# anihcsam/OpenGaussian

Measured on AMD Instinct MI355X. Metric: fwd+bwd Mpix/s at 1080p, 1M Gaussians (RGB+6-D ins_feat); k-means it/s, higher is better.
Workload: dtype f32; 1 GPU; S1M-1080p RGB(SH3)+depth+alpha (all grads) + 6-ch ins_feat (grad to ins_feat) fwd+bwd, ONE fused 9-channel pass; gaussians=1000000, width=1920, height=1080, views_cycled=8, parallelism=single

## Files before the change

include/ogs_raster.h:

```cpp
#ifndef OGS_RASTER_H
#define OGS_RASTER_H

#include <stddef.h>
#include <stdint.h>

#ifdef __cplusplus
extern "C" {
#endif

#define OGS_OK 0
#define OGS_ERR_INVALID_ARG (-1)
#define OGS_ERR_HIP (-2)
#define OGS_ERR_UNSUPPORTED (-3)
#define OGS_ERR_SCRATCH_TOO_SMALL (-4)
#define OGS_ERR_DEVICE (-5)

#define OGS_TILE 16
#define OGS_MAX_CHANNELS 12

typedef struct OgsRasterFwdArgs {
    int32_t P;
    int32_t W, H;
    int32_t C;
    int32_t sh_degree;
// ... 69 lines not shown
    float* dL_drotations;
    int32_t num_groups;
    float* dL_dsh_rgb;
    int32_t bwd_tmp_is_clear;
} OgsRasterBwdArgs;

int ogs_version(void);
const char* ogs_last_error(void);

int ogs_check_async_status(void);

size_t ogs_raster_geom_bytes(int32_t P, int32_t C);
size_t ogs_raster_geom_tmp_bytes(int32_t P);
size_t ogs_raster_image_bytes(int32_t W, int32_t H);
size_t ogs_raster_image_bytes_grouped(int32_t W, int32_t H, int32_t num_groups);
size_t ogs_raster_binning_tmp_bytes(int64_t num_rendered, int32_t W, int32_t H);
size_t ogs_raster_backward_tmp_bytes(int32_t P);
size_t ogs_raster_sorted_bytes(int64_t num_rendered, int32_t C);
size_t ogs_raster_quad_list_bytes(int64_t num_rendered);

int ogs_raster_forward_geometry(const OgsRasterFwdArgs* args, void* stream, int64_t* num_rendered_host);

int ogs_raster_forward_render(const OgsRasterFwdArgs* args, int64_t num_rendered, void* stream);

int ogs_raster_read_num_rendered_async(const OgsRasterFwdArgs* args, void* stream, uint32_t* host_pinned);
int ogs_raster_forward_render_deferred(const OgsRasterFwdArgs* args, int64_t capacity, void* stream);

int ogs_raster_read_num_emitted(const OgsRasterFwdArgs* args, void* stream, uint32_t* host);

size_t ogs_raster_tiny_max_points(void);
int ogs_raster_forward_tiny(const OgsRasterFwdArgs* args, void* stream);

size_t ogs_raster_tile_sort_capacity(int32_t level);

int ogs_raster_tile_count_debug(int64_t D, int64_t tiles, int32_t force_blocks, int32_t reverse);
size_t ogs_raster_tile_count_trip(void);

int ogs_raster_tile_place_debug(int64_t D, int64_t tiles, int32_t group, int32_t slices, int32_t stage_words, int32_t* chosen);

int ogs_raster_forward_reblend(const OgsRasterFwdArgs* args, void* stream);

int ogs_raster_compact_kept(int32_t W, int32_t H, int32_t C, const void* image_buffer, const void* sorted_rec,
                            const void* quad_list, void* new_image_buffer, void* new_sorted_rec, void* new_quad_list,
                            void* stream);

typedef struct OgsGroupStatsArgs {
    const int32_t* labels;
    int32_t num_labels;
    float alpha_threshold;
    float* max_alpha;
    int64_t* count;
    float* feat_sum;
    void* stats_tmp;
} OgsGroupStatsArgs;

size_t ogs_raster_stats_image_bytes(int32_t W, int32_t H, int32_t num_groups);
size_t ogs_raster_stats_tmp_bytes(int32_t num_groups, int32_t num_labels, int32_t C);
int ogs_raster_forward_group_stats(const OgsRasterFwdArgs* args, const OgsGroupStatsArgs* stats, int64_t num_rendered,
                                   void* stream);

int ogs_raster_backward(const OgsRasterBwdArgs* args, void* stream);

int ogs_mark_visible(int32_t P, const float* means3D, const float* viewmatrix, const float* projmatrix,
                     uint8_t* present, void* stream);

int ogs_sh_grad_from_views(int32_t P, int32_t V, int32_t sh_degree, int32_t sh_coeffs, const float* means3D,
// ... 23 lines not shown
```

opengaussian_amd/_lib.py:

```python
from __future__ import annotations

import ctypes as C
import os

_HERE = os.path.dirname(os.path.abspath(__file__))
LIB_PATH = os.environ.get("OGS_LIB_PATH") or os.path.join(_HERE, "lib", "libogs_hip.so")

_f32p = C.POINTER(C.c_float)
_vp = C.c_void_p


class OgsRasterFwdArgs(C.Structure):
    _fields_ = [
        ("P", C.c_int32), ("W", C.c_int32), ("H", C.c_int32), ("C", C.c_int32),
        ("sh_degree", C.c_int32), ("sh_coeffs", C.c_int32),
        ("tanfovx", C.c_float), ("tanfovy", C.c_float), ("scale_modifier", C.c_float),
        ("prefiltered", C.c_int32), ("debug", C.c_int32),
        ("bg", _vp), ("means3D", _vp), ("colors_precomp", _vp), ("shs", _vp), ("opacities", _vp),
        ("scales", _vp), ("rotations", _vp), ("cov3D_precomp", _vp),
        ("viewmatrix", _vp), ("projmatrix", _vp), ("campos", _vp),
        ("out_color", _vp), ("out_depth", _vp), ("out_alpha", _vp), ("radii", _vp),
        ("geom_buffer", _vp), ("geom_tmp", _vp), ("image_buffer", _vp), ("point_list", _vp),
        ("binning_tmp", _vp), ("sorted_rec", _vp), ("quad_list", _vp), ("group_ids", _vp), ("num_groups", C.c_int32),
        ("full_binning", C.c_int32),
# ... 57 lines not shown
                ("channels_last", C.c_int32), ("out_map", _vp), ("out_alpha", _vp)]


class OgsRawModel(C.Structure):
    _fields_ = [("features_dc", _vp), ("features_rest", _vp), ("scaling", _vp), ("rotation", _vp), ("opacity", _vp)]


class OgsRawModelGrads(C.Structure):
    _fields_ = [("features_dc", _vp), ("features_rest", _vp), ("scaling", _vp), ("rotation", _vp), ("opacity", _vp)]


SIGNATURES = {
    "ogs_version": (C.c_int, []),
    "ogs_last_error": (C.c_char_p, []),
    "ogs_raster_geom_bytes": (C.c_size_t, [C.c_int32, C.c_int32]),
    "ogs_raster_geom_tmp_bytes": (C.c_size_t, [C.c_int32]),
    "ogs_raster_image_bytes": (C.c_size_t, [C.c_int32, C.c_int32]),
    "ogs_raster_image_bytes_grouped": (C.c_size_t, [C.c_int32, C.c_int32, C.c_int32]),
    "ogs_raster_binning_tmp_bytes": (C.c_size_t, [C.c_int64, C.c_int32, C.c_int32]),
    "ogs_raster_backward_tmp_bytes": (C.c_size_t, [C.c_int32]),
    "ogs_raster_sorted_bytes": (C.c_size_t, [C.c_int64, C.c_int32]),
    "ogs_raster_quad_list_bytes": (C.c_size_t, [C.c_int64]),
    "ogs_raster_forward_geometry": (C.c_int, [C.POINTER(OgsRasterFwdArgs), _vp, C.POINTER(C.c_int64)]),
    "ogs_raster_forward_render": (C.c_int, [C.POINTER(OgsRasterFwdArgs), C.c_int64, _vp]),
    "ogs_raster_read_num_rendered_async": (C.c_int, [C.POINTER(OgsRasterFwdArgs), _vp, _vp]),
    "ogs_raster_forward_render_deferred": (C.c_int, [C.POINTER(OgsRasterFwdArgs), C.c_int64, _vp]),
    "ogs_raster_read_num_emitted": (C.c_int, [C.POINTER(OgsRasterFwdArgs), _vp, C.POINTER(C.c_uint32)]),
    "ogs_raster_stats_image_bytes": (C.c_size_t, [C.c_int32, C.c_int32, C.c_int32]),
    "ogs_raster_stats_tmp_bytes": (C.c_size_t, [C.c_int32, C.c_int32, C.c_int32]),
    "ogs_raster_forward_group_stats": (C.c_int, [C.POINTER(OgsRasterFwdArgs), C.POINTER(OgsGroupStatsArgs), C.c_int64, _vp]),
    "ogs_raster_backward": (C.c_int, [C.POINTER(OgsRasterBwdArgs), _vp]),
    "ogs_raster_tiny_max_points": (C.c_size_t, []),
    "ogs_raster_tile_sort_capacity": (C.c_size_t, [C.c_int32]),
    "ogs_raster_tile_count_debug": (C.c_int, [C.c_int64, C.c_int64, C.c_int32, C.c_int32]),
    "ogs_raster_tile_count_trip": (C.c_size_t, []),
    "ogs_raster_tile_place_debug": (C.c_int, [C.c_int64, C.c_int64, C.c_int32, C.c_int32, C.c_int32, C.POINTER(C.c_int32)]),
    "ogs_raster_forward_tiny": (C.c_int, [C.POINTER(OgsRasterFwdArgs), _vp]),
    "ogs_raster_forward_reblend": (C.c_int, [C.POINTER(OgsRasterFwdArgs), _vp]),
    "ogs_raster_compact_kept": (C.c_int, [C.c_int32, C.c_int32, C.c_int32, _vp, _vp, _vp, _vp, _vp, _vp, _vp]),
    "ogs_mark_visible": (C.c_int, [C.c_int32, _vp, _vp, _vp, _vp, _vp]),
    "ogs_sh_grad_from_views": (C.c_int, [C.c_int32, C.c_int32, C.c_int32, C.c_int32, _vp, _vp, _vp, _vp, _vp]),
    "ogs_raster_export_binning": (C.c_int, [C.POINTER(OgsRasterFwdArgs), C.c_int64, _vp, _vp, _vp, _vp]),
    "ogs_selftest_wave_fold16": (C.c_int, [_vp, _vp, _vp]),
    "ogs_selftest_mfma_rank1": (C.c_int, [_vp, _vp, _vp, C.c_int32, _vp, _vp, _vp]),
    "ogs_selftest_tile_order": (C.c_int, [_vp, C.c_int64, _vp, _vp]),
    "ogs_selftest_radix_tmp_bytes": (C.c_size_t, [C.c_int64]),
    "ogs_selftest_radix_sort": (C.c_int, [_vp, _vp, _vp, _vp, C.c_int64, C.c_int32, C.c_int32, C.c_int32, _vp, _vp, _vp, _vp]),
    "ogs_raster_forward_geometry_raw": (C.c_int, [C.POINTER(OgsRasterFwdArgs), C.POINTER(OgsRawModel), _vp,
                                                  C.POINTER(C.c_int64)]),
    "ogs_raster_forward_tiny_raw": (C.c_int, [C.POINTER(OgsRasterFwdArgs), C.POINTER(OgsRawModel), _vp]),
    "ogs_raster_backward_raw": (C.c_int, [C.POINTER(OgsRasterBwdArgs), C.POINTER(OgsRawModel), C.POINTER(OgsRawModelGrads), _vp]),
    "ogs_model_activate": (C.c_int, [C.c_int32, C.c_int32, C.POINTER(OgsRawModel), _vp, _vp, _vp, _vp, _vp]),
    "ogs_check_async_status": (C.c_int, []),
    "ogs_prof_enable": (C.c_int, [C.c_int]),
    "ogs_prof_filter": (C.c_int, [C.c_char_p]),
    "ogs_prof_collect": (C.c_int, [C.c_char_p, C.c_size_t]),
    "ogs_kmeans_tmp_bytes": (C.c_size_t, [C.c_int64, C.c_int32, C.c_int32]),
    "ogs_kmeans_lloyd": (C.c_int, [_vp, C.c_int64, C.c_int32, _vp, C.c_int32, C.c_int32, C.c_int32, C.c_int32,
                                   _vp, C.c_int64, _vp, _vp]),
    "ogs_kmeans_assign": (C.c_int, [_vp, C.c_int64, C.c_int32, _vp, C.c_int32, _vp, C.c_int64, _vp]),
    "ogs_mask_feature_sums": (C.c_int, [_vp, _vp, _vp, C.c_int32, C.c_int32, C.c_int64, C.c_int32, _vp, _vp]),
    "ogs_mask_feature_sqdev": (C.c_int, [_vp, _vp, _vp, _vp, C.c_int32, C.c_int32, C.c_int64, _vp, _vp]),
    "ogs_mask_feature_sums_backward": (C.c_int, [_vp, _vp, _vp, _vp, _vp, C.c_int32, C.c_int32, C.c_int64, _vp, _vp, _vp]),
    "ogs_mask_cohesion": (C.c_int, [_vp, _vp, _vp, C.c_int32, C.c_int32, C.c_int64, _vp, _vp]),
    "ogs_mask_cohesion_backward": (C.c_int, [_vp, _vp, _vp, _vp, C.c_int32, C.c_int32, C.c_int64, _vp, _vp, _vp]),
    "ogs_label_feature_sums": (C.c_int, [_vp, _vp, _vp, C.c_int32, C.c_int32, C.c_int64, C.c_int32, _vp, _vp]),
# ... 151 lines not shown
```

opengaussian_amd/csrc/binning.hip:

```cpp
#include <stdlib.h>
#include <string.h>

#include <atomic>

#include "ogs_common.h"

namespace ogs {

namespace {

constexpr size_t kSweepHeaderWords = 4 * 256 + 4 + 60;
constexpr int kScanItems = 8;
constexpr int kScanTile = kBlock * kScanItems;

__device__ __forceinline__ uint32_t wave_inclusive_scan(uint32_t v) {
#pragma unroll
    for (int d = 1; d < kWave; d <<= 1) {
        uint32_t t = __shfl_up(v, d, kWave);
        if (lane_id() >= d) v += t;
    }
    return v;
}

__device__ __forceinline__ uint32_t block_exclusive_scan(uint32_t v, uint32_t& total, uint32_t* wave_sums ) {
    const int wave = threadIdx.x >> 6;
    const uint32_t inc = wave_inclusive_scan(v);
    if (lane_id() == kWave - 1) wave_sums[wave] = inc;
    __syncthreads();
    uint32_t base = 0, tot = 0;
#pragma unroll
    for (int w = 0; w < kBlock / kWave; ++w) {
        const uint32_t s = wave_sums[w];
// ... 613 lines not shown
        run_mine += c;
    }
    if (p == 0 && blockIdx.y == gridDim.y - 1 && threadIdx.x == 0) *kept = total;
    if (begin >= end || nt == 0 || (may_stage && need == 0)) return;
    __syncthreads();
    for (int j = threadIdx.x; j < nt; j += kCountBlock) (staged ? delta : cur)[j] += row[j];
    __syncthreads();
    const uint32_t ulo = (uint32_t)t_lo, unt = (uint32_t)nt;
    uint16_t* stile = reinterpret_cast<uint16_t*>(stage + stage_words);
    if (!staged) {
        tile_place_walk<false>(keys, vals, begin, end, reverse, ulo, unt, cur, stage, stile, stage_words, out, out_cap);
        return;
    }
    tile_place_walk<true>(keys, vals, begin, end, reverse, ulo, unt, cur, stage, stile, stage_words, out, out_cap);
    __syncthreads();
    for (uint32_t i = threadIdx.x; i < need; i += kCountBlock) {
        const uint32_t pos = delta[min((int)stile[i], nt - 1)] + i;
        if (pos < out_cap) out[pos] = stage[i];
    }
}

constexpr int kTileSortWaves = kBlock / kWave;
struct TileSortLds {
    uint32_t hist[kTileSortWaves][256];
    uint32_t dig_start[256];
    uint32_t base[256];
    uint32_t scan_sums[4];
    uint32_t red[2];
    uint2 range[kTileSortWaves];
    uint32_t kv[2 * kTileSortCap];
};
typedef __attribute__((address_space(3))) volatile uint32_t LdsWord;
typedef __attribute__((address_space(3))) unsigned long long LdsMask;
__device__ __forceinline__ LdsWord* lds_words(uint32_t* p) { return (LdsWord*)p; }
__device__ __forceinline__ LdsMask* wave_masks(TileSortLds& sm, int wave) { return (LdsMask*)(sm.kv + wave * 2 * kWaveSortCap); }

__device__ __forceinline__ void wave_rank_clear(LdsWord* hist, LdsMask* masks) {
    const int lane = threadIdx.x & (kWave - 1);
#pragma unroll
    for (int j = 0; j < 4; ++j) {
        hist[lane + j * kWave] = 0u;
        __hip_atomic_store(&masks[lane + j * kWave], 0ull, __ATOMIC_SEQ_CST, __HIP_MEMORY_SCOPE_WAVEFRONT);
    }
    __builtin_amdgcn_wave_barrier();
}

__device__ __forceinline__ void wave_rank(LdsWord* hist, LdsMask* masks, const uint32_t (&key)[kTileSortItems],
                                          uint32_t (&rank)[kTileSortItems], int ipl, int first, int m, int shift,
                                          uint32_t mask) {
    const int lane = threadIdx.x & (kWave - 1);
    const unsigned long long me = 1ull << lane;
#pragma unroll
    for (int i = 0; i < kTileSortItems; ++i) {
        if (i >= ipl) continue;
        const bool valid = first + i * kWave + lane < m;
        const uint32_t d = (key[i] >> shift) & mask;
        if (valid) __hip_atomic_fetch_or(&masks[d], me, __ATOMIC_SEQ_CST, __HIP_MEMORY_SCOPE_WAVEFRONT);
        __builtin_amdgcn_wave_barrier();
        const unsigned long long peers =
            valid ? __hip_atomic_load(&masks[d], __ATOMIC_SEQ_CST, __HIP_MEMORY_SCOPE_WAVEFRONT) : 0ull;
        const uint32_t r = __builtin_amdgcn_mbcnt_hi((uint32_t)(peers >> 32), __builtin_amdgcn_mbcnt_lo((uint32_t)peers, 0u));
        uint32_t pre = 0;
        if (valid) pre = hist[d];
        __builtin_amdgcn_wave_barrier();
        if (valid && r == 0) {
            hist[d] = pre + (uint32_t)__popcll(peers);
// ... 79 lines not shown
#pragma unroll
        for (int j = 0; j < 4; ++j) { c[j] = hist[4 * lane + j]; sum += c[j]; }
        uint32_t run = wave_inclusive_scan(sum) - sum;
#pragma unroll
        for (int j = 0; j < 4; ++j) { hist[4 * lane + j] = run; run += c[j]; }
        __builtin_amdgcn_wave_barrier();
#pragma unroll
        for (int i = 0; i < kTileSortItems; ++i) {
            if (i >= ipl) continue;
            rank[i] += hist[(sel[i] >> shift) & mask];
        }
#pragma unroll
        for (int i = 0; i < kTileSortItems; ++i) {
            if (i >= ipl) continue;
            if (i * kWave + lane < n) {
                wk[rank[i]] = key[i];
                wv[rank[i]] = val[i];
            }
        }
        __builtin_amdgcn_wave_barrier();
        if (p + 1 < npass || reload_last) {
#pragma unroll
            for (int i = 0; i < kTileSortItems; ++i) {
                if (i >= ipl) continue;
                const int e = min(i * kWave + lane, n - 1);
                key[i] = wk[e];
                val[i] = wv[e];
            }
            __builtin_amdgcn_wave_barrier();
        }
    }
}

__device__ __forceinline__ void wave_sort_list(TileSortLds& sm, uint32_t* __restrict__ seg, int n,
                                               const uint32_t* __restrict__ depth_keys) {
    const int lane = threadIdx.x & (kWave - 1), wave = threadIdx.x >> 6;
    LdsWord* wk = lds_words(sm.kv + wave * 2 * kWaveSortCap);
    LdsWord* wv = wk + kWaveSortCap;
    LdsWord* hist = lds_words(sm.hist[wave]);
    LdsMask* masks = wave_masks(sm, wave);
    uint32_t key[kTileSortItems], val[kTileSortItems], rank[kTileSortItems];
    const int ipl = (n + kWave - 1) / kWave;
    load_items(seg, depth_keys, key, val, ipl, lane, n);
    uint32_t k_and, k_or;
    wave_and_or(key, ipl, 0xFFFFFFFFu, k_and, k_or);
    const uint32_t kdiff = (uint32_t)__builtin_amdgcn_readfirstlane((int)(k_and ^ k_or));
    if (kdiff != 0u) {
        wave_lsd_passes(hist, masks, wk, wv, key, key, val, rank, ipl, n, kdiff, false);
    } else {
#pragma unroll
        for (int i = 0; i < kTileSortItems; ++i) {
            if (i >= ipl) continue;
            if (i * kWave + lane < n) { wk[i * kWave + lane] = key[i]; wv[i * kWave + lane] = val[i]; }
        }
        __builtin_amdgcn_wave_barrier();
    }
    bool bad = false;
#pragma unroll
    for (int i = 0; i < kTileSortItems; ++i) {
        if (i >= ipl) continue;
        const int e = min(i * kWave + lane, n - 2);
        if (wk[e] == wk[e + 1]) bad |= (wv[e] & kGidMask) > (wv[e + 1] & kGidMask);
    }
    if (__ballot(bad) != 0ull) {
#pragma unroll
        for (int i = 0; i < kTileSortItems; ++i) {
            if (i >= ipl) continue;
            const int e = min(i * kWave + lane, n - 1);
            key[i] = wk[e];
            val[i] = wv[e];
        }
        __builtin_amdgcn_wave_barrier();
        wave_and_or(val, ipl, kGidMask, k_and, k_or);
        const uint32_t gdiff = (uint32_t)__builtin_amdgcn_readfirstlane((int)(k_and ^ k_or));
        if (gdiff != 0u) wave_lsd_passes(hist, masks, wk, wv, val, key, val, rank, ipl, n, gdiff, kdiff != 0u);
        if (kdiff != 0u) wave_lsd_passes(hist, masks, wk, wv, key, key, val, rank, ipl, n, kdiff, false);
    } else if (kdiff == 0u) {
        return;
    }
// ... 161 lines not shown
            return;
        }
        for (int j = tid; j < n; j += kBlock) seg[j] = sv[j];
        return;
    }

    uint32_t k_and = 0xFFFFFFFFu, k_or = 0u;
    for (int j = tid; j < n; j += kBlock) {
        const uint32_t k = depth_keys[seg[j] & kGidMask];
        k_and &= k;
        k_or |= k;
    }
    const uint32_t kdiff = block_and_or(sm, k_and, k_or, any);
    if (kdiff != 0u) long_lsd_passes<false>(sm, seg, alt, n, depth_keys, kdiff);
    bool bad = false;
    k_and = 0xFFFFFFFFu; k_or = 0u;
    for (int j = tid; j < n; j += kBlock) {
        const uint32_t v0 = seg[j], v1 = seg[min(j + 1, n - 1)];
        bad |= tie_out_of_order(depth_keys[v0 & kGidMask], v0, depth_keys[v1 & kGidMask], v1);
        k_and &= v0 & kGidMask;
        k_or |= v0 & kGidMask;
    }
    const uint32_t gdiff = block_and_or(sm, k_and, k_or | (bad ? 0x80000000u : 0u), any) & kGidMask;
    if ((any & 0x80000000u) == 0u || gdiff == 0u) return;
    long_lsd_passes<true>(sm, seg, alt, n, depth_keys, gdiff);
    if (kdiff != 0u) long_lsd_passes<false>(sm, seg, alt, n, depth_keys, kdiff);
}


__global__ __launch_bounds__(kBlock) void tile_depth_sort_kernel(const uint2* __restrict__ ranges, int tiles,
                                                                 const uint32_t* __restrict__ tile_order,
                                                                 uint32_t* __restrict__ point_list,
                                                                 const uint32_t* __restrict__ depth_keys,
                                                                 uint32_t* __restrict__ scratch) {
    __shared__ TileSortLds sm;
    const int wave = threadIdx.x >> 6;
    if (threadIdx.x < kTileSortWaves) {
        const int b = blockIdx.x * kTileSortWaves + threadIdx.x;
        sm.range[threadIdx.x] = b < tiles ? ranges[tile_order ? tile_order[b] : (uint32_t)b] : make_uint2(0u, 0u);
    }
    __syncthreads();
    const uint32_t x = (uint32_t)__builtin_amdgcn_readfirstlane((int)sm.range[wave].x);
    const int n = __builtin_amdgcn_readfirstlane((int)(sm.range[wave].y - sm.range[wave].x));
    if (n >= 2 && n <= kWaveSortCap) wave_sort_list(sm, point_list + x, n, depth_keys);
#pragma unroll 1
    for (int w = 0; w < kTileSortWaves; ++w) {
        const uint32_t xw = (uint32_t)__builtin_amdgcn_readfirstlane((int)sm.range[w].x);
        const int nw = __builtin_amdgcn_readfirstlane((int)(sm.range[w].y - sm.range[w].x));
        if (nw > kWaveSortCap) block_sort_list(sm, point_list + xw, scratch + xw, nw, depth_keys);
    }
}

__global__ __launch_bounds__(kBlock) void export_keys_kernel(const uint2* __restrict__ ranges,
                                                             const uint32_t* __restrict__ point_list,
                                                             const float4* __restrict__ rec, int recv4,
                                                             uint64_t* __restrict__ keys_out) {
    const uint32_t tile = blockIdx.x;
    const uint2 r = ranges[tile];
    for (uint32_t i = r.x + threadIdx.x; i < r.y; i += kBlock) {
        const uint32_t gid = point_list[i] & kGidMask;
        const uint32_t bits = __float_as_uint(rec[(size_t)gid * recv4].z);
        keys_out[i] = ((uint64_t)tile << 32) | bits;
    }
}

}

size_t scan_tmp_bytes(int64_t n) {
    size_t total = 0;
    int64_t m = n;
    while (true) {
        const int nb = scan_blocks(m);
        if (nb <= 1) break;
        total += align_up((size_t)nb * sizeof(uint32_t));
        m = nb;
    }
    return total + kAlign;
// ... 211 lines not shown
}

int launch_tile_count_binning(const uint32_t* keys, const uint32_t* vals, int64_t D, const uint32_t* n_dev, int B, int64_t tiles,
                              uint32_t* table, uint2* ranges, uint32_t* kept, uint32_t* point_list, hipStream_t s, int debug) {
    if (B < 1 || tiles < 1 || tiles > kTileCountMaxTiles || ((int64_t)B + 1) * tiles > D) {
        set_error("tile_count_binning: B=%d tiles=%lld D=%lld", B, (long long)tiles, (long long)D); return OGS_ERR_INVALID_ARG;
    }
    const size_t lds = (size_t)tiles * sizeof(uint32_t);
    OGS_LAUNCH(tile_count_kernel, dim3(B), dim3(kCountBlock), lds, s, keys, D, n_dev, (int)tiles, table);
    OGS_LAUNCH_CHECK(debug, s);
    const int cols = (int)((tiles + kCountScanCols - 1) / kCountScanCols);
    OGS_LAUNCH(tile_count_scan_kernel, dim3(cols), dim3(kCountScanCols * kCountScanGroups), 0, s, table, B, (int)tiles);
    OGS_LAUNCH_CHECK(debug, s);
    const TilePlacePlan pl = tile_place_plan(D, tiles, B);
    const size_t per_slice = (size_t)((tiles + pl.slices - 1) / pl.slices);
    const size_t place_lds = pl.stage_words ? (8 * per_slice + (size_t)kPlaceEntryBytes * pl.stage_words + 15) / 16 * 16
                                            : per_slice * sizeof(uint32_t);
    if (place_lds > 48 * 1024) {
        static std::atomic<bool> raised[64];
        int dev = 0;
        OGS_HIP_CHECK(hipGetDevice(&dev));
        if (dev < 0 || dev >= 64 || !raised[dev].load(std::memory_order_relaxed)) {
            OGS_HIP_CHECK(hipFuncSetAttribute(reinterpret_cast<const void*>(tile_place_kernel),
                                              hipFuncAttributeMaxDynamicSharedMemorySize, (int)kPlaceLdsBytes));
            if (dev >= 0 && dev < 64) raised[dev].store(true, std::memory_order_relaxed);
        }
    }
    OGS_LAUNCH(tile_place_kernel, dim3(pl.chunks, pl.slices), dim3(kCountBlock), place_lds, s, keys, vals, D, n_dev, (int)tiles, B,
               pl.group, pl.stage_words, (const uint32_t*)table, ranges, kept, point_list, (uint32_t)D, g_tile_place_reverse);
    OGS_LAUNCH_CHECK(debug, s);
    return OGS_OK;
}

int launch_tile_depth_sort(const uint2* ranges, int64_t tiles, const uint32_t* tile_order, uint32_t* point_list,
                           const uint32_t* depth_keys, uint32_t* scratch, hipStream_t s, int debug) {
    if (tiles <= 0) return OGS_OK;
    if (tiles >= (1ll << 31)) { set_error("tile_depth_sort: %lld tiles", (long long)tiles); return OGS_ERR_UNSUPPORTED; }
    const unsigned grid = (unsigned)((tiles + kTileSortWaves - 1) / kTileSortWaves);
    OGS_LAUNCH(tile_depth_sort_kernel, dim3(grid), dim3(kBlock), 0, s, ranges, (int)tiles, tile_order, point_list, depth_keys,
               scratch);
    OGS_LAUNCH_CHECK(debug, s);
    return OGS_OK;
}

int launch_export_keys(const uint2* ranges, int tiles, const uint32_t* point_list, const float4* rec, int recv4,
                       uint64_t* keys_out, hipStream_t s) {
    OGS_LAUNCH(export_keys_kernel, dim3(tiles), dim3(kBlock), 0, s, ranges, point_list, rec, recv4, keys_out);
    OGS_LAUNCH_CHECK(0, s);
    return OGS_OK;
}

}
```

opengaussian_amd/csrc/capi.hip:

```cpp
#include <stdarg.h>
#include <stdlib.h>
#include <string.h>

#include <map>
#include <mutex>
#include <string>
#include <vector>

#include "ogs_common.h"

namespace ogs {

static thread_local char g_err[512] = "";

void set_error(const char* fmt, ...) {
    va_list ap;
    va_start(ap, fmt);
    vsnprintf(g_err, sizeof(g_err), fmt, ap);
    va_end(ap);
}

namespace {
struct ProfRec { const char* name; hipEvent_t start, stop; };
int g_prof_mode = 0;
// ... 118 lines not shown
    if (M < 1) { set_error("raw model: sh_coeffs=%d < 1", M); return OGS_ERR_INVALID_ARG; }
    if (P > 0 && (!raw->features_dc || !raw->scaling || !raw->rotation || !raw->opacity)) {
        set_error("raw model: NULL features_dc / scaling / rotation / opacity"); return OGS_ERR_INVALID_ARG;
    }
    if (P > 0 && M > 1 && !raw->features_rest) { set_error("raw model: features_rest == NULL with %d SH coefficients", M); return OGS_ERR_INVALID_ARG; }
    return OGS_OK;
}

static int raw_fwd_args(const OgsRasterFwdArgs* a, const OgsRawModel* raw, OgsRasterFwdArgs* out) {
    if (!a) { set_error("args == NULL"); return OGS_ERR_INVALID_ARG; }
    if (a->shs || a->opacities || a->scales || a->rotations || a->cov3D_precomp) {
        set_error("raw pass: args.shs / opacities / scales / rotations / cov3D_precomp must be NULL (the raw model takes their place)");
        return OGS_ERR_INVALID_ARG;
    }
    int rc = validate_raw(raw, a->P, a->sh_coeffs);
    if (rc != OGS_OK) return rc;
    *out = *a;
    out->shs = raw->features_dc;
    out->opacities = raw->opacity;
    out->scales = raw->scaling;
    out->rotations = raw->rotation;
    if (a->P == 0) {
        out->shs = out->scales = out->rotations = a->bg;
    }
    return OGS_OK;
}

}

using namespace ogs;

extern "C" {

int ogs_version(void) { return 410; }

int ogs_check_async_status(void) { return check_async_status("ogs_check_async_status"); }

int ogs_prof_enable(int on) {
    std::lock_guard<std::mutex> lk(g_prof_mu);
    for (auto& r : g_prof) { g_event_pool.push_back(r.start); g_event_pool.push_back(r.stop); }
    g_prof.clear();
    g_prof_mode = on;
    return OGS_OK;
}

int ogs_prof_filter(const char* prefix) {
    std::lock_guard<std::mutex> lk(g_prof_mu);
    if (!prefix || strlen(prefix) >= sizeof(g_prof_prefix)) { set_error("prof_filter: prefix NULL or longer than %zu", sizeof(g_prof_prefix) - 1); return OGS_ERR_INVALID_ARG; }
    strcpy(g_prof_prefix, prefix);
    return OGS_OK;
}

int ogs_prof_collect(char* buf, size_t n) {
    std::lock_guard<std::mutex> lk(g_prof_mu);
    std::map<std::string, std::pair<long, double>> agg;
    for (auto& r : g_prof) {
        OGS_HIP_CHECK(hipEventSynchronize(r.stop));
        float ms = 0.f;
        OGS_HIP_CHECK(hipEventElapsedTime(&ms, r.start, r.stop));
        auto& a = agg[r.name];
        a.first += 1;
        a.second += ms;
    }
    std::string out = "{";
    bool first = true;
    for (auto& kv : agg) {
        char line[384];
// ... 230 lines not shown
}

int ogs_raster_forward_reblend(const OgsRasterFwdArgs* a, void* stream_) {
    if (!a) { set_error("args == NULL"); return OGS_ERR_INVALID_ARG; }
    if (a->P <= 0 || a->W <= 0 || a->H <= 0) { set_error("forward_reblend: bad sizes P=%d W=%d H=%d", a->P, a->W, a->H); return OGS_ERR_INVALID_ARG; }
    if (a->C != 3 && a->C != 6 && a->C != 9 && a->C != 12) { set_error("C=%d unsupported (3, 6, 9, 12)", a->C); return OGS_ERR_UNSUPPORTED; }
    if (a->num_groups > 1) { set_error("forward_reblend: grouped passes are not kept"); return OGS_ERR_UNSUPPORTED; }
    if (!a->colors_precomp || !a->bg || !a->out_color || !a->out_depth || !a->out_alpha || !a->image_buffer || !a->sorted_rec ||
        !a->quad_list) {
        set_error("forward_reblend: NULL required pointer (colors_precomp, bg, out_*, image_buffer, sorted_rec, quad_list)");
        return OGS_ERR_INVALID_ARG;
    }
    const int rc = check_async_status("forward_reblend (entry)");
    if (rc != OGS_OK) return rc;
    const ImageState is = ImageState::carve(a->image_buffer, a->W, a->H, 1);
    return launch_reblend(*a, is, static_cast<hipStream_t>(stream_));
}

int ogs_raster_compact_kept(int32_t W, int32_t H, int32_t C, const void* image_buffer, const void* sorted_rec, const void* quad_list,
                            void* new_image_buffer, void* new_sorted_rec, void* new_quad_list, void* stream_) {
    if (W <= 0 || H <= 0) { set_error("compact_kept: bad sizes W=%d H=%d", W, H); return OGS_ERR_INVALID_ARG; }
    if (!image_buffer || !sorted_rec || !quad_list || !new_image_buffer || !new_sorted_rec || !new_quad_list) {
        set_error("compact_kept: NULL pointer"); return OGS_ERR_INVALID_ARG;
    }
    const ImageState is_old = ImageState::carve(const_cast<void*>(image_buffer), W, H, 1);
    const ImageState is_new = ImageState::carve(new_image_buffer, W, H, 1);
    return launch_compact_kept(W, H, C, is_old, is_new, sorted_rec, quad_list, new_sorted_rec, new_quad_list,
                               static_cast<hipStream_t>(stream_));
}

size_t ogs_raster_tiny_max_points(void) { return (size_t)kTinyMaxP; }

size_t ogs_raster_tile_sort_capacity(int32_t level) {
    return level == 0 ? (size_t)kWaveSortCap : level == 1 ? (size_t)kTileSortCap : 0;
}

int ogs_raster_tile_count_debug(int64_t D, int64_t tiles, int32_t force_blocks, int32_t reverse) {
    tile_count_debug(force_blocks, reverse);
    return tile_count_blocks(D, tiles);
}
size_t ogs_raster_tile_count_trip(void) { return (size_t)tile_count_trip(); }

int ogs_raster_tile_place_debug(int64_t D, int64_t tiles, int32_t group, int32_t slices, int32_t stage_words, int32_t* chosen) {
    tile_place_debug(group, slices, stage_words);
    if (chosen) {
        const TilePlacePlan pl = tile_place_plan(D, tiles, tile_count_blocks(D, tiles));
        chosen[0] = pl.chunks; chosen[1] = pl.slices; chosen[2] = (int32_t)pl.stage_words;
    }
    return OGS_OK;
}

static int forward_tiny_impl(const OgsRasterFwdArgs* a_in, void* stream_, bool raw, const float* raw_rest) {
    int rc = validate_fwd(a_in);
    if (rc != OGS_OK) return rc;
    OgsRasterFwdArgs a_raw;
    const OgsRasterFwdArgs* a = a_in;
    if (raw) { a_raw = *a_in; a_raw.cov3D_precomp = raw_rest; a = &a_raw; }
    if (a->P <= 0 || a->P > kTinyMaxP) { set_error("forward_tiny: P=%d outside [1, %d]", a->P, kTinyMaxP); return OGS_ERR_INVALID_ARG; }
    if (a->num_groups > 1) { set_error("forward_tiny: grouped passes use the streaming path"); return OGS_ERR_UNSUPPORTED; }
    hipStream_t s = static_cast<hipStream_t>(stream_);
    const GeomState gs = GeomState::carve(a->geom_buffer, a->P, a->C);
    uint32_t* order = static_cast<uint32_t*>(a->geom_tmp);
    rc = launch_tiny_geometry(*a, gs, order, s, raw);
    if (rc != OGS_OK) return rc;
    return launch_tiny_blend(*a, gs, order, s);
}

// ... 181 lines not shown
```

opengaussian_amd/csrc/ogs_common.h:

```cpp
#pragma once

#include <hip/hip_runtime.h>
#include <stdint.h>
#include <stddef.h>
#include <stdio.h>
#include <type_traits>

#include "../../include/ogs_raster.h"
#include "../../include/ogs_model.h"

namespace ogs {

constexpr int kTile = OGS_TILE;
constexpr int kBlock = 256;
constexpr int kWave = 64;
constexpr int kTinyMaxP = 256;
constexpr int kSmallMaxP = 1024;

void set_error(const char* fmt, ...);

#define OGS_HIP_CHECK(expr)                                                              \
    do {                                                                                 \
        hipError_t _e = (expr);                                                          \
        if (_e != hipSuccess) {                                                          \
// ... 252 lines not shown
    }
};

int launch_preprocess(const OgsRasterFwdArgs& a, const GeomState& gs, const GeomTmp& gt, hipStream_t s, bool raw = false);
int launch_block_offsets(const OgsRasterFwdArgs& a, const GeomTmp& gt, hipStream_t s);
int launch_tiny_geometry(const OgsRasterFwdArgs& a, const GeomState& gs, uint32_t* order, hipStream_t s, bool raw = false);
int launch_small_geometry(const OgsRasterFwdArgs& a, const GeomState& gs, const GeomTmp& gt, hipStream_t s, bool raw = false);
int launch_model_activate(int P, int M, const OgsRawModel& raw, float* scales, float* rotations, float* opacities, float* shs,
                          hipStream_t s);
int launch_tiny_blend(const OgsRasterFwdArgs& a, const GeomState& gs, const uint32_t* order, hipStream_t s);
int launch_reblend(const OgsRasterFwdArgs& a, const ImageState& is, hipStream_t s);
int launch_compact_kept(int W, int H, int C, const ImageState& is_old, const ImageState& is_new, const void* old_rec,
                        const void* old_quad, void* new_rec, void* new_quad, hipStream_t s);
int launch_duplicate(const OgsRasterFwdArgs& a, const GeomState& gs, const GeomTmp& gt, uint32_t* tile_keys,
                     uint32_t* vals, uint32_t capacity, bool drop_unreachable, bool depth_order, hipStream_t s,
                     uint2* zero_ranges = nullptr, int n_zero = 0);
int launch_tile_ranges(const uint32_t* tile_keys_sorted, int64_t D, uint2* ranges, int64_t tiles, hipStream_t s,
                       int debug, const uint32_t* n_dev = nullptr, bool already_zeroed = false);
constexpr int kTileCountMaxTiles = 12288;
constexpr int kTileCountBlocks = 128;
int tile_count_blocks(int64_t D, int64_t tiles);
int tile_count_trip();
void tile_count_debug(int force_blocks, int reverse);
struct TilePlacePlan { int group, chunks, slices; uint32_t stage_words; };
TilePlacePlan tile_place_plan(int64_t D, int64_t tiles, int B);
void tile_place_debug(int group, int slices, int stage_words);
int launch_tile_count_binning(const uint32_t* keys, const uint32_t* vals, int64_t D, const uint32_t* n_dev, int B, int64_t tiles,
                              uint32_t* table, uint2* ranges, uint32_t* kept, uint32_t* point_list, hipStream_t s, int debug);
inline bool per_tile_depth_order(const OgsRasterFwdArgs& a) { return a.num_groups <= 1 && a.P > kSmallMaxP; }
inline bool block_sum_offsets(const OgsRasterFwdArgs& a) { return per_tile_depth_order(a) && a.full_binning == 0; }
constexpr int kTileSortItems = 16;
constexpr int kTileSortCap = kBlock * kTileSortItems;
constexpr int kWaveSortCap = kTileSortCap / (kBlock / kWave);
int launch_tile_depth_sort(const uint2* ranges, int64_t tiles, const uint32_t* tile_order, uint32_t* point_list,
                           const uint32_t* depth_keys, uint32_t* scratch, hipStream_t s, int debug);
inline int num_groups_of(int g) { return g > 1 ? g : 1; }
int launch_group_stats(const OgsRasterFwdArgs& a, const OgsGroupStatsArgs& st, const GeomState& gs, const ImageState& is,
                       hipStream_t s, bool order_ready = false);
int launch_blend_forward(const OgsRasterFwdArgs& a, const GeomState& gs, const ImageState& is, int64_t D,
                         hipStream_t s, bool order_ready = false);
int launch_blend_backward(const OgsRasterBwdArgs& a, const ImageState& is, void* grad_rec, hipStream_t s);
int launch_preprocess_backward(const OgsRasterBwdArgs& a, const GeomState& gs, const void* grad_rec, hipStream_t s,
                               const OgsRawModelGrads* raw_grads = nullptr);
inline bool backward_is_features_only(const OgsRasterBwdArgs& a) {
    return a.dL_dcolors != nullptr && a.colors_precomp != nullptr && !a.dL_dmeans2D && !a.dL_dopacity &&
           !a.dL_dmeans3D && !a.dL_dcov3D && !a.dL_dsh && !a.dL_dscales && !a.dL_drotations && !a.dL_dsh_rgb;
}
int launch_sh_grad_from_views(int P, int V, int sh_degree, int sh_coeffs, const float* means3D, const float* campos,
                              const float* dL_drgb, float* dL_dsh, hipStream_t s);
int launch_wave_fold16_test(const float* in, float* out, hipStream_t s);
int launch_mfma_rank1_test(const float* w, const float* f, const float* acc0, int steps, float* out_mfma, float* out_fma,
                           hipStream_t s);
int launch_tile_order_test(const uint32_t* ranges, int64_t vtiles, uint32_t* order, hipStream_t s);
int launch_mark_visible(int P, const float* means3D, const float* viewmatrix, uint8_t* present, hipStream_t s);
int launch_export_keys(const uint2* ranges, int tiles, const uint32_t* point_list, const float4* rec, int recv4,
                       uint64_t* keys_out, hipStream_t s);

__device__ __forceinline__ float blend_power(float a2, float b2, float c2, float dx, float dy) {
    const float u = fmaf(b2, dy, a2 * dx);
    return fmaf(c2 * dy, dy, u * dx);
}

constexpr int kPrefetchMax = 4;
struct RecordPrefetch {
    uint32_t v[kPrefetchMax];
    __device__ __forceinline__ void issue(const float* __restrict__ tile_records, int n_tile, int rec_floats, int tid,
// ... 45 lines not shown
```

Baseline: 1557 Mpix/s.

## Add bucket-rank wave sort path for per-tile depth ordering

Adds a per-wave bucket-rank sort used in the tile depth sort before the LSD radix passes. Keys are bucketed into 256 buckets by their leading bits over the wave's min/max range, then ranked within each bucket by pairwise comparison, and the sort falls back to LSD passes when any bucket exceeds a cap (default 32). The aim is to replace several radix passes with one histogram plus short comparison loops for typical tile lists. The cost is extra LDS traffic, roughly quadratic work in bucket size, and more register pressure. Debug hooks for the cap and compile-time experiment switches are also added.

Measured after the change: 1579 Mpix/s (median of 6 runs). 1.01x the previous value.

```diff
diff --git a/include/ogs_raster.h b/include/ogs_raster.h
--- a/include/ogs_raster.h
+++ b/include/ogs_raster.h
@@ -125,6 +125,7 @@
 int ogs_raster_forward_tiny(const OgsRasterFwdArgs* args, void* stream);
 
 size_t ogs_raster_tile_sort_capacity(int32_t level);
+int ogs_raster_tile_sort_debug(int32_t bucket_cap);
 
 int ogs_raster_tile_count_debug(int64_t D, int64_t tiles, int32_t force_blocks, int32_t reverse);
 size_t ogs_raster_tile_count_trip(void);
diff --git a/opengaussian_amd/_lib.py b/opengaussian_amd/_lib.py
--- a/opengaussian_amd/_lib.py
+++ b/opengaussian_amd/_lib.py
@@ -113,6 +113,7 @@
     "ogs_raster_backward": (C.c_int, [C.POINTER(OgsRasterBwdArgs), _vp]),
     "ogs_raster_tiny_max_points": (C.c_size_t, []),
     "ogs_raster_tile_sort_capacity": (C.c_size_t, [C.c_int32]),
+    "ogs_raster_tile_sort_debug": (C.c_int, [C.c_int32]),
     "ogs_raster_tile_count_debug": (C.c_int, [C.c_int64, C.c_int64, C.c_int32, C.c_int32]),
     "ogs_raster_tile_count_trip": (C.c_size_t, []),
     "ogs_raster_tile_place_debug": (C.c_int, [C.c_int64, C.c_int64, C.c_int32, C.c_int32, C.c_int32, C.POINTER(C.c_int32)]),
diff --git a/opengaussian_amd/csrc/binning.hip b/opengaussian_amd/csrc/binning.hip
--- a/opengaussian_amd/csrc/binning.hip
+++ b/opengaussian_amd/csrc/binning.hip
@@ -1,3 +1,4 @@
+#include <stddef.h>
 #include <stdlib.h>
 #include <string.h>
 
@@ -677,6 +678,7 @@
 };
 typedef __attribute__((address_space(3))) volatile uint32_t LdsWord;
 typedef __attribute__((address_space(3))) unsigned long long LdsMask;
+static_assert(offsetof(TileSortLds, kv) % 8 == 0, "a wave's quarter of kv is read as 64-bit pairs");
 __device__ __forceinline__ LdsWord* lds_words(uint32_t* p) { return (LdsWord*)p; }
 __device__ __forceinline__ LdsMask* wave_masks(TileSortLds& sm, int wave) { return (LdsMask*)(sm.kv + wave * 2 * kWaveSortCap); }
 
@@ -822,8 +824,137 @@
     }
 }
 
+#if defined(OGS_EXPERIMENTS) && defined(OGS_TSORT_LOADS_ONLY)
+constexpr bool kTsortLoadsOnly = true;
+#else
+constexpr bool kTsortLoadsOnly = false;
+#endif
+#if defined(OGS_EXPERIMENTS) && defined(OGS_TSORT_SKIP_PASSES)
+constexpr bool kTsortSkipPasses = true;
+#else
+constexpr bool kTsortSkipPasses = false;
+#endif
+#if defined(OGS_EXPERIMENTS) && defined(OGS_TSORT_LSD_ONLY)
+constexpr bool kTsortLsdOnly = true;
+#else
+constexpr bool kTsortLsdOnly = false;
+#endif
+
+__device__ __forceinline__ void wave_min_max(const uint32_t (&w)[kTileSortItems], int ipl, uint32_t keep, uint32_t& w_min,
+                                             uint32_t& w_max) {
+    w_min = 0xFFFFFFFFu; w_max = 0u;
+#pragma unroll
+    for (int i = 0; i < kTileSortItems; ++i) {
+        if (i >= ipl) continue;
+        w_min = min(w_min, w[i] & keep);
+        w_max = max(w_max, w[i] & keep);
+    }
+#pragma unroll
+    for (int d = 32; d >= 1; d >>= 1) {
+        w_min = min(w_min, (uint32_t)__shfl_xor((int)w_min, d, kWave));
+        w_max = max(w_max, (uint32_t)__shfl_xor((int)w_max, d, kWave));
+    }
+}
+
+typedef __attribute__((address_space(3))) uint32_t LdsCount;
+typedef __attribute__((address_space(3))) volatile unsigned long long LdsPair;
+
+constexpr int kRankGroup = 8;
+template <int IPL>
+__device__ __forceinline__ void bucket_rank_steps(LdsPair* pairs, const unsigned long long (&mine)[kTileSortItems],
+                                                  const uint32_t (&st)[kTileSortItems], uint32_t (&cw)[kTileSortItems], int cmax,
+                                                  int n) {
+#pragma unroll 1
+    for (int t = 0; t < cmax; ++t) {
+        const uint32_t tt = ((uint32_t)t << 16) | 0xFFFFu;
+#pragma unroll
+        for (int g = 0; g < IPL; g += kRankGroup) {
+            unsigned long long other[kRankGroup];
+#pragma unroll
+            for (int i = g; i < min(IPL, g + kRankGroup); ++i)
+                other[i - g] = pairs[min((int)st[i] + t, n - 1)];
+#pragma unroll
+            for (int i = g; i < min(IPL, g + kRankGroup); ++i)
+                cw[i] += (tt < cw[i] && other[i - g] < mine[i]) ? 1u : 0u;
+        }
+    }
+}
+
+constexpr int kBucketBits = 8;
+__device__ __forceinline__ bool wave_bucket_rank(LdsWord* hist, LdsWord* wk, LdsWord* wv, const uint32_t (&key)[kTileSortItems],
+                                                 const uint32_t (&val)[kTileSortItems], int ipl, int n, int bucket_cap) {
+    const int lane = threadIdx.x & (kWave - 1);
+    uint32_t w_min, w_max;
+    wave_min_max(key, ipl, 0xFFFFFFFFu, w_min, w_max);
+    const bool by_id = __builtin_amdgcn_readfirstlane((int)w_min) == __builtin_amdgcn_readfirstlane((int)w_max);
+    if (by_id) wave_min_max(val, ipl, kGidMask, w_min, w_max);
+    const uint32_t base = (uint32_t)__builtin_amdgcn_readfirstlane((int)w_min);
+    const uint32_t range = (uint32_t)__builtin_amdgcn_readfirstlane((int)w_max) - base;
+    if (range == 0u) return false;
+    const int shift = max(0, 32 - __builtin_clz(range) - kBucketBits);
+#pragma unroll
+    for (int j = 0; j < 4; ++j) hist[lane + j * kWave] = 0u;
+    __builtin_amdgcn_wave_barrier();
+    uint32_t slot[kTileSortItems];
+#pragma unroll
+    for (int i = 0; i < kTileSortItems; ++i) {
+        if (i >= ipl) continue;
+        const uint32_t d = ((by_id ? val[i] & kGidMask : key[i]) - base) >> shift;
+        slot[i] = 0u;
+        if (i * kWave + lane < n)
+            slot[i] = __hip_atomic_fetch_add((LdsCount*)(hist + d), 1u, __ATOMIC_RELAXED, __HIP_MEMORY_SCOPE_WAVEFRONT);
+    }
+    __builtin_amdgcn_wave_barrier();
+    uint32_t c[4], sum = 0, big = 0;
+#pragma unroll
+    for (int j = 0; j < 4; ++j) { c[j] = hist[4 * lane + j]; sum += c[j]; big = max(big, c[j]); }
+    uint32_t run = wave_inclusive_scan(sum) - sum;
+#pragma unroll
+    for (int d = 32; d >= 1; d >>= 1) big = max(big, (uint32_t)__shfl_xor((int)big, d, kWave));
+    const int cmax = __builtin_amdgcn_readfirstlane((int)big);
+    if (cmax > bucket_cap) return false;
+#pragma unroll
+    for (int j = 0; j < 4; ++j) { hist[4 * lane + j] = run | (c[j] << 10); run += c[j]; }
+    __builtin_amdgcn_wave_barrier();
+    LdsPair* pairs = (LdsPair*)wk;
+    unsigned long long mine[kTileSortItems];
+    uint32_t st[kTileSortItems], cw[kTileSortItems];
+#pragma unroll
+    for (int i = 0; i < kTileSortItems; ++i) {
+        if (i >= ipl) continue;
+        slot[i] = hist[((by_id ? val[i] & kGidMask : key[i]) - base) >> shift] | (slot[i] << 21);
+    }
+#pragma unroll
+    for (int i = 0; i < kTileSortItems; ++i) {
+        uint32_t s_i = 0u, c_i = 0u;
+        unsigned long long m_i = 0ull;
+        if (i < ipl) {
+            const bool valid = i * kWave + lane < n;
+            c_i = valid ? ((slot[i] >> 10) & 0x7FFu) << 16 : 0u;
+            s_i = slot[i] & 0x3FFu;
+            m_i = ((unsigned long long)key[i] << 32) | (unsigned long long)((val[i] << 1) | (val[i] >> 31));
+            if (valid) pairs[s_i + (slot[i] >> 21)] = m_i;
+        }
+        st[i] = s_i; cw[i] = c_i; mine[i] = m_i;
+    }
+    __builtin_amdgcn_wave_barrier();
+    if (ipl <= 4) bucket_rank_steps<4>(pairs, mine, st, cw, cmax, n);
+    else if (ipl <= 8) bucket_rank_steps<8>(pairs, mine, st, cw, cmax, n);
+    else if (ipl <= 12) bucket_rank_steps<12>(pairs, mine, st, cw, cmax, n);
+    else bucket_rank_steps<kTileSortItems>(pairs, mine, st, cw, cmax, n);
+    __builtin_amdgcn_wave_barrier();
+#pragma unroll
+    for (int i = 0; i < kTileSortItems; ++i) {
+        if (i >= ipl) continue;
+        const uint32_t w = (uint32_t)mine[i];
+        if (i * kWave + lane < n) wv[st[i] + (cw[i] & 0xFFFFu)] = (w >> 1) | (w << 31);
+    }
+    __builtin_amdgcn_wave_barrier();
+    return true;
+}
+
 __device__ __forceinline__ void wave_sort_list(TileSortLds& sm, uint32_t* __restrict__ seg, int n,
-                                               const uint32_t* __restrict__ depth_keys) {
+                                               const uint32_t* __restrict__ depth_keys, int bucket_cap) {
     const int lane = threadIdx.x & (kWave - 1), wave = threadIdx.x >> 6;
     LdsWord* wk = lds_words(sm.kv + wave * 2 * kWaveSortCap);
     LdsWord* wv = wk + kWaveSortCap;
@@ -835,6 +966,24 @@
     uint32_t k_and, k_or;
     wave_and_or(key, ipl, 0xFFFFFFFFu, k_and, k_or);
     const uint32_t kdiff = (uint32_t)__builtin_amdgcn_readfirstlane((int)(k_and ^ k_or));
+    if (kTsortLoadsOnly) {
+        if (kdiff == 0x5A5A5A5Au) seg[0] = key[0];
+        return;
+    }
+    if (kTsortSkipPasses) {
+#pragma unroll
+        for (int i = 0; i < kTileSortItems; ++i) {
+            if (i >= ipl) continue;
+            if (i * kWave + lane < n) { wk[i * kWave + lane] = key[i]; wv[i * kWave + lane] = val[i]; }
+        }
+        __builtin_amdgcn_wave_barrier();
+        for (int j = lane; j < n; j += kWave) seg[j] = wv[j];
+        return;
+    }
+    if (!kTsortLsdOnly && wave_bucket_rank(hist, wk, wv, key, val, ipl, n, bucket_cap)) {
+        for (int j = lane; j < n; j += kWave) seg[j] = wv[j];
+        return;
+    }
     if (kdiff != 0u) {
         wave_lsd_passes(hist, masks, wk, wv, key, key, val, rank, ipl, n, kdiff, false);
     } else {
@@ -1062,7 +1211,7 @@
                                                                  const uint32_t* __restrict__ tile_order,
                                                                  uint32_t* __restrict__ point_list,
                                                                  const uint32_t* __restrict__ depth_keys,
-                                                                 uint32_t* __restrict__ scratch) {
+                                                                 uint32_t* __restrict__ scratch, int bucket_cap) {
     __shared__ TileSortLds sm;
     const int wave = threadIdx.x >> 6;
     if (threadIdx.x < kTileSortWaves) {
@@ -1072,7 +1221,7 @@
     __syncthreads();
     const uint32_t x = (uint32_t)__builtin_amdgcn_readfirstlane((int)sm.range[wave].x);
     const int n = __builtin_amdgcn_readfirstlane((int)(sm.range[wave].y - sm.range[wave].x));
-    if (n >= 2 && n <= kWaveSortCap) wave_sort_list(sm, point_list + x, n, depth_keys);
+    if (n >= 2 && n <= kWaveSortCap) wave_sort_list(sm, point_list + x, n, depth_keys, bucket_cap);
 #pragma unroll 1
     for (int w = 0; w < kTileSortWaves; ++w) {
         const uint32_t xw = (uint32_t)__builtin_amdgcn_readfirstlane((int)sm.range[w].x);
@@ -1350,13 +1499,19 @@
     return OGS_OK;
 }
 
+static int g_tile_sort_bucket_cap = 0;
+void tile_sort_debug(int bucket_cap) {
+    if (bucket_cap >= 0) g_tile_sort_bucket_cap = bucket_cap;
+}
+int tile_sort_bucket_cap() { return g_tile_sort_bucket_cap > 0 ? g_tile_sort_bucket_cap : kWaveBucketCap; }
+
 int launch_tile_depth_sort(const uint2* ranges, int64_t tiles, const uint32_t* tile_order, uint32_t* point_list,
                            const uint32_t* depth_keys, uint32_t* scratch, hipStream_t s, int debug) {
     if (tiles <= 0) return OGS_OK;
     if (tiles >= (1ll << 31)) { set_error("tile_depth_sort: %lld tiles", (long long)tiles); return OGS_ERR_UNSUPPORTED; }
     const unsigned grid = (unsigned)((tiles + kTileSortWaves - 1) / kTileSortWaves);
     OGS_LAUNCH(tile_depth_sort_kernel, dim3(grid), dim3(kBlock), 0, s, ranges, (int)tiles, tile_order, point_list, depth_keys,
-               scratch);
+               scratch, tile_sort_bucket_cap());
     OGS_LAUNCH_CHECK(debug, s);
     return OGS_OK;
 }
diff --git a/opengaussian_amd/csrc/capi.hip b/opengaussian_amd/csrc/capi.hip
--- a/opengaussian_amd/csrc/capi.hip
+++ b/opengaussian_amd/csrc/capi.hip
@@ -174,7 +174,7 @@
 
 extern "C" {
 
-int ogs_version(void) { return 410; }
+int ogs_version(void) { return 420; }
 
 int ogs_check_async_status(void) { return check_async_status("ogs_check_async_status"); }
 
@@ -471,7 +471,12 @@
 size_t ogs_raster_tiny_max_points(void) { return (size_t)kTinyMaxP; }
 
 size_t ogs_raster_tile_sort_capacity(int32_t level) {
-    return level == 0 ? (size_t)kWaveSortCap : level == 1 ? (size_t)kTileSortCap : 0;
+    return level == 0 ? (size_t)kWaveSortCap : level == 1 ? (size_t)kTileSortCap : level == 2 ? (size_t)tile_sort_bucket_cap() : 0;
+}
+
+int ogs_raster_tile_sort_debug(int32_t bucket_cap) {
+    tile_sort_debug(bucket_cap);
+    return OGS_OK;
 }
 
 int ogs_raster_tile_count_debug(int64_t D, int64_t tiles, int32_t force_blocks, int32_t reverse) {
diff --git a/opengaussian_amd/csrc/ogs_common.h b/opengaussian_amd/csrc/ogs_common.h
--- a/opengaussian_amd/csrc/ogs_common.h
+++ b/opengaussian_amd/csrc/ogs_common.h
@@ -308,6 +308,9 @@
 constexpr int kTileSortItems = 16;
 constexpr int kTileSortCap = kBlock * kTileSortItems;
 constexpr int kWaveSortCap = kTileSortCap / (kBlock / kWave);
+constexpr int kWaveBucketCap = 32;
+void tile_sort_debug(int bucket_cap);
+int tile_sort_bucket_cap();
 int launch_tile_depth_sort(const uint2* ranges, int64_t tiles, const uint32_t* tile_order, uint32_t* point_list,
                            const uint32_t* depth_keys, uint32_t* scratch, hipStream_t s, int debug);
 inline int num_groups_of(int g) { return g > 1 ? g : 1; }
```
